# dscripka/openWakeWord

Measured on NVIDIA B200. Metric: 80ms audio-frames/sec (concurrent streams), higher is better.
Workload: dtype f16 operands / f32 accumulate (mel, BN, LayerNorm, sigmoid in f32; heads' first layer as fp16 hi/lo split = f32-grade)

## Files before the change

### openwakeword_b200/csrc/cnn_tc_inc.cu

```cuda
#include "oww_internal.h"
#include "tc_common.cuh"
#include "mel_device.cuh"
#include <cstring>

namespace {

constexpr int kIncEpiWarps = 16;
constexpr int kIncThreads = (kIncEpiWarps + 2) * 32;
constexpr int kIncAcc = 4;
constexpr int kIncMaxG = 7;
constexpr int kMelNF = 2;

__device__ __forceinline__ __half2 u32_as_half2(uint32_t v) {
    return __halves2half2(__ushort_as_half((unsigned short)(v & 0xFFFFu)), __ushort_as_half((unsigned short)(v >> 16)));
}
__device__ __forceinline__ bool elect_one() {
    uint32_t pred;
    asm volatile("{\n\t.reg .pred p;\n\telect.sync _|p, 0xffffffff;\n\tselp.u32 %0, 1, 0, p;\n\t}" : "=r"(pred));
    return pred != 0;
}
__device__ __forceinline__ void named_bar_sync(int id, int n) { asm volatile("bar.sync %0, %1;" ::"r"(id), "r"(n) : "memory"); }
__device__ __forceinline__ void tmem_ld8(uint32_t taddr, uint32_t* v) {
    asm volatile("tcgen05.ld.sync.aligned.32x32b.x8.b32 {%0,%1,%2,%3,%4,%5,%6,%7}, [%8];"
                 : "=r"(v[0]), "=r"(v[1]), "=r"(v[2]), "=r"(v[3]), "=r"(v[4]), "=r"(v[5]), "=r"(v[6]), "=r"(v[7])
// ... 184 lines not shown
                            for (int q = 0; q < nq; ++q) {
                                const uint32_t alo = (q < n_pair ? a_hi_pair : a_hi_self) | ((a_tap + (uint32_t)q * pitch2) & 0x3FFFu);
                                const uint32_t blo = b_lo0 | ((b_tap + (uint32_t)q * np2) & 0x3FFFu);
                                tc_mma_f16(d_tmem, dhi | alo, dhi | blo, idesc, accumulate);
                                accumulate = 1;
                            }
                        }
                        }
                        tc_commit(tfull(acc));
                    }
                    __syncwarp();
                    if (++acc == kIncAcc) { acc = 0; acc_par ^= 1; }
                }
                if (dbg) a.dbg_clock[41 + l] = clock64() - c0;
                have_prev = true; prev_i = i;
                __syncwarp();
            }
        }
    } else {
        const int et = threadIdx.x;
        const int quarter = warp & 3, part = warp >> 2;
        const int row = quarter * 32 + lane;
        int acc = 0; uint32_t acc_par = 0;
        uint32_t epar[2] = {0, 0};
        uint32_t epi_tails_par = 0;
        uint32_t hf_par = 0; int hchunk_e = 0;
        for (int grp = blockIdx.x; grp < P.n_groups; grp += gridDim.x) {
            const uint4* tin = a.tails_in + (int64_t)grp * P.tail_units;
            uint4* tout = a.tails_out + (int64_t)grp * P.tail_units;
            int* s_cnt = reinterpret_cast<int*>(smem + 512);
            int* s_live = s_cnt + 16;
            float* s_mel = reinterpret_cast<float*>(smem + P.scratch_off + 6144);
            if (a.dbg_clock && blockIdx.x == 0 && grp == 0 && et == 0) a.dbg_clock[101] = clock64();
            named_bar_sync(2, kIncEpiWarps * 32);
            if (et < G) {
                const int b = grp * G + et;
                s_live[et] = b < a.B;
            }
            named_bar_sync(2, kIncEpiWarps * 32);
            if (a.fused) {
                uint8_t* sc = smem + P.scratch_off;
                float2* s_tw = reinterpret_cast<float2*>(sc);
                float* s_win = reinterpret_cast<float*>(sc + 4096);
                uint8_t* s_work = smem + 2048 + warp * (kMelNF * kMelFrameScratch);
                float* s_floor = s_mel + G * 256;
                int seen_v = 1;
                for (int i = et; i < 512; i += kIncEpiWarps * 32) { s_tw[i] = a.mel_twiddle[i]; s_win[i] = a.mel_window[i]; }
                if (et < G) {
                    const int b = grp * G + et;
                    s_cnt[et] = s_live[et] ? a.mel_count_rw[b] : 0;
                    s_cnt[8 + et] = s_live[et] ? a.feat_count[b] : 0;
                    seen_v = s_live[et] ? a.seen[b] : 1;
                    s_live[8 + et] = s_live[et] && seen_v == 0;
                }
                named_bar_sync(2, kIncEpiWarps * 32);
                const int my_start = a.mel_start[lane], my_len = a.mel_len[lane];
                const float* my_w = a.mel_w + lane * OWW_MEL_MAXSUPPORT;
                for (int fi = warp * kMelNF; fi < G * 8; fi += kIncEpiWarps * kMelNF) {
                    const int16_t* tl[kMelNF]; const int16_t* bd[kMelNF]; int fr[kMelNF]; float db[kMelNF];
#pragma unroll
                    for (int i = 0; i < kMelNF; ++i) {
                        const int fj = fi + i < G * 8 ? fi + i : fi;
                        int b = grp * G + (fj >> 3);
                        if (b >= a.B) b = grp * G;
                        tl[i] = a.tail + (int64_t)b * OWW_TAIL; bd[i] = a.pcm + (int64_t)b * a.pcm_stride; fr[i] = fj & 7;
                    }
                    long long* st = (a.dbg_clock && blockIdx.x == 0 && grp == 0 && warp == 0 && fi == 0) ? a.dbg_clock + 92 : nullptr;
                    mel_frames_db<kMelNF>(tl, OWW_TAIL, bd, fr, s_work, s_tw, s_win, a.mel_kmax, my_start, my_len, my_w, lane, db, st);
#pragma unroll
                    for (int i = 0; i < kMelNF; ++i)
                        if (fi + i < G * 8) s_mel[(fi + i) * 32 + lane] = db[i];
                }
                named_bar_sync(2, kIncEpiWarps * 32);
                if (a.dbg_clock && blockIdx.x == 0 && grp == 0 && et == 0) a.dbg_clock[97] = clock64();
                constexpr int kTW = OWW_TAIL / 2;
                const bool al = ((size_t)a.pcm & 3) == 0 && (a.pcm_stride & 1) == 0;
                uint32_t tv[4]; int ti[4];
#pragma unroll
                for (int u = 0; u < 4; ++u) {
                    const int i = et + u * kIncEpiWarps * 32;
                    ti[u] = -1; tv[u] = 0;
                    if (i < G * kTW) {
                        const int g = i / kTW, k = i - g * kTW, b = grp * G + g;
                        if (s_live[g]) {
                            const int16_t* src = a.pcm + (int64_t)b * a.pcm_stride + (OWW_SAMPLES_PER_CHUNK - OWW_TAIL) + 2 * k;
                            tv[u] = al ? __ldg(reinterpret_cast<const uint32_t*>(src))
                                       : ((uint32_t)(unsigned short)__ldg(src) | ((uint32_t)(unsigned short)__ldg(src + 1) << 16));
                            ti[u] = b * kTW + k;
// ... 859 lines not shown
```

### openwakeword_b200/csrc/mel_device.cuh

```cuda
#pragma once
#include <cuda_runtime.h>
#include <cstdint>
#include "oww_internal.h"

namespace {

__device__ __forceinline__ float2 cmul(float2 a, float2 b) {
    return make_float2(__fmaf_rn(a.x, b.x, -__fmul_rn(a.y, b.y)), __fmaf_rn(a.x, b.y, __fmul_rn(a.y, b.x)));
}

template <bool kBodyGlobal = true>
__device__ __forceinline__ float mel_frame_db(const int16_t* tail, int prefix, const int16_t* body, int f, float2* a, float2* b,
                                              float* pw_buf, const float2* s_tw, const float* s_win, int kmax, int my_start,
                                              int my_len, const float* my_w, int lane) {
#pragma unroll
        for (int j = 0; j < 8; ++j) {
            const int n = lane + 32 * j;
            const int s0 = f * OWW_HOP + 2 * n;
            float x0, x1;
            if (s0 + 1 < prefix) { x0 = (float)tail[s0]; x1 = (float)tail[s0 + 1]; }
            else if (s0 >= prefix) {
                if (kBodyGlobal) { x0 = (float)__ldg(body + (s0 - prefix)); x1 = (float)__ldg(body + (s0 + 1 - prefix)); }
                else { x0 = (float)body[s0 - prefix]; x1 = (float)body[s0 + 1 - prefix]; }
            }
// ... 67 lines not shown
                                              uint8_t* bufs, const float2* s_tw, const float* s_win, int kmax, int my_start,
                                              int my_len, const float* my_w, int lane, float* db, long long* stamps = nullptr) {
    float2* a[NF]; float2* b[NF]; float* pw[NF];
    if (stamps && lane == 0) stamps[0] = clock64();
#pragma unroll
    for (int i = 0; i < NF; ++i) {
        a[i] = reinterpret_cast<float2*>(bufs + i * kMelFrameScratch);
        b[i] = a[i] + 256;
        pw[i] = reinterpret_cast<float*>(b[i] + 256);
    }
    bool al[NF];
#pragma unroll
    for (int i = 0; i < NF; ++i) al[i] = (((size_t)body[i] | (size_t)tail[i]) & 3) == 0 && (prefix & 1) == 0;
    uint32_t raw[8][NF];
#pragma unroll
    for (int j = 0; j < 8; ++j) {
        const int n = lane + 32 * j;
#pragma unroll
        for (int i = 0; i < NF; ++i) {
            const int s0 = f[i] * OWW_HOP + 2 * n;
            if (al[i]) {
                raw[j][i] = s0 + 1 < prefix ? *reinterpret_cast<const uint32_t*>(tail[i] + s0)
                                            : __ldg(reinterpret_cast<const uint32_t*>(body[i] + (s0 - prefix)));
            } else {
                unsigned short u0, u1;
                if (s0 + 1 < prefix) { u0 = (unsigned short)tail[i][s0]; u1 = (unsigned short)tail[i][s0 + 1]; }
                else if (s0 >= prefix) { u0 = (unsigned short)__ldg(body[i] + (s0 - prefix)); u1 = (unsigned short)__ldg(body[i] + (s0 + 1 - prefix)); }
                else { u0 = (unsigned short)tail[i][s0]; u1 = (unsigned short)__ldg(body[i]); }
                raw[j][i] = (uint32_t)u0 | ((uint32_t)u1 << 16);
            }
        }
    }
#pragma unroll
    for (int j = 0; j < 8; ++j) {
        const int n = lane + 32 * j;
        const float2 wn = *reinterpret_cast<const float2*>(s_win + 2 * n);
#pragma unroll
        for (int i = 0; i < NF; ++i) {
            const float x0 = (float)(short)(raw[j][i] & 0xFFFFu), x1 = (float)(short)(raw[j][i] >> 16);
            a[i][fswz(n)] = make_float2(__fmul_rn(x0, wn.x), __fmul_rn(x1, wn.y));
        }
    }
    __syncwarp();
    if (stamps && lane == 0) stamps[1] = clock64();
#pragma unroll
    for (int Ns = 1; Ns < 256; Ns *= 4) {
        const int tstep = 128 / Ns;
        float2 t1 = make_float2(1.f, 0.f), t2 = t1, t3 = t1;
        if (Ns > 1 && Ns <= 32) { const int k = lane & (Ns - 1); t1 = s_tw[k * tstep]; t2 = s_tw[2 * k * tstep]; t3 = s_tw[3 * k * tstep]; }
#pragma unroll
        for (int jj = 0; jj < 2; ++jj) {
            const int j = lane + 32 * jj;
            const int k = j & (Ns - 1);
            if (Ns > 32) { t1 = s_tw[k * tstep]; t2 = s_tw[2 * k * tstep]; t3 = s_tw[3 * k * tstep]; }
            const int dst = (j / Ns) * Ns * 4 + k;
            const int sj = fswz(j);
            const int d0 = fswz(dst), d1 = fswz(dst + Ns), d2 = fswz(dst + 2 * Ns), d3 = fswz(dst + 3 * Ns);
#pragma unroll
            for (int i = 0; i < NF; ++i) {
                const float2 v0 = a[i][sj];
                float2 v1 = a[i][sj + 64], v2 = a[i][sj + 128], v3 = a[i][sj + 192];
                if (Ns > 1) { v1 = cmul(v1, t1); v2 = cmul(v2, t2); v3 = cmul(v3, t3); }
                float2 a0 = make_float2(v0.x + v2.x, v0.y + v2.y);
                float2 a1 = make_float2(v0.x - v2.x, v0.y - v2.y);
                float2 a2 = make_float2(v1.x + v3.x, v1.y + v3.y);
                float2 d = make_float2(v1.x - v3.x, v1.y - v3.y);
                float2 a3 = make_float2(d.y, -d.x);
                b[i][d0] = make_float2(a0.x + a2.x, a0.y + a2.y);
                b[i][d1] = make_float2(a1.x + a3.x, a1.y + a3.y);
                b[i][d2] = make_float2(a0.x - a2.x, a0.y - a2.y);
                b[i][d3] = make_float2(a1.x - a3.x, a1.y - a3.y);
            }
        }
        __syncwarp();
#pragma unroll
        for (int i = 0; i < NF; ++i) { float2* t = a[i]; a[i] = b[i]; b[i] = t; }
    }
    if (stamps && lane == 0) stamps[2] = clock64();
    for (int k = lane; k < kmax; k += 32) {
#pragma unroll
        for (int i = 0; i < NF; ++i) {
            float p;
            if (k == 256) {
                const float x = a[i][fswz(0)].x - a[i][fswz(0)].y;
                p = __fmul_rn(x, x);
            } else {
                const float2 zk = a[i][fswz(k & 255)];
                const float2 zc = a[i][fswz((256 - k) & 255)];
                const float2 xe = make_float2(0.5f * (zk.x + zc.x), 0.5f * (zk.y - zc.y));
                const float2 dd = make_float2(zk.x - zc.x, zk.y + zc.y);
                const float2 xo = make_float2(0.5f * dd.y, -0.5f * dd.x);
                const float2 t2 = cmul(s_tw[k], xo);
                const float re = __fadd_rn(xe.x, t2.x), im = __fadd_rn(xe.y, t2.y);
                p = __fmaf_rn(re, re, __fmul_rn(im, im));
            }
// ... 26 lines not shown
```

### openwakeword_b200/csrc/api.cu

```cuda
#include "oww_internal.h"
#include <cstdarg>
#include <cstdlib>
#include <cstring>
#include <algorithm>

static thread_local std::string g_create_error;

int oww_fail(oww_ctx* ctx, int code, const char* fmt, ...) {
    char buf[512];
    va_list ap;
    va_start(ap, fmt);
    vsnprintf(buf, sizeof(buf), fmt, ap);
    va_end(ap);
    if (ctx) ctx->err = buf; else g_create_error = buf;
    return code;
}

namespace {

const int kLayerTable[OWW_N_CONV][6] = {
    {3, 3, 1, 24, 0, 0},
    {1, 3, 24, 24, 0, 0}, {3, 1, 24, 24, 2, 2},
    {1, 3, 24, 48, 0, 0}, {3, 1, 48, 48, 0, 0},
    {1, 3, 48, 48, 0, 0}, {3, 1, 48, 48, 1, 2},
// ... 139 lines not shown
        const int r = (int)((i / 24) % n_rows);
        const int64_t clip = i / ((int64_t)24 * n_rows);
        reinterpret_cast<float4*>(feats + clip * clip_stride + (int64_t)r * 96)[c4] =
            init ? __ldg(reinterpret_cast<const float4*>(init + (int64_t)r * 96) + c4) : make_float4(0.f, 0.f, 0.f, 0.f);
    }
}

int ensure_emb_tmp(oww_ctx* ctx, size_t floats) {
    if (ctx->emb_tmp_floats >= floats) return OWW_OK;
    cudaFree(ctx->d_emb_tmp); ctx->d_emb_tmp = nullptr; ctx->emb_tmp_floats = 0;
    OWW_CUDA(ctx, cudaMalloc(&ctx->d_emb_tmp, floats * sizeof(float)));
    ctx->emb_tmp_floats = floats;
    return OWW_OK;
}

int step_core(oww_ctx* ctx, const int16_t* d_pcm, int64_t pcm_stride, int n_chunks, float* d_scores, int out_stride,
              cudaStream_t s) {
    const int B = ctx->n_streams;
    if (B <= 0) return oww_fail(ctx, OWW_EINVAL, "oww_set_streams has not been called");
    if (n_chunks < 1 || n_chunks > ctx->cfg.max_chunks)
        return oww_fail(ctx, OWW_EINVAL, "n_chunks=%d outside [1,%d]", n_chunks, ctx->cfg.max_chunks);
    if (!ctx->mel_loaded || !ctx->emb_loaded) return oww_fail(ctx, OWW_EINVAL, "weights not loaded");
    int rc;
    const long slot = ctx->timing ? ctx->ev_steps % ctx->ev_slots : 0;
    cudaEvent_t* ev = ctx->timing ? &ctx->ev[4 * slot] : nullptr;
    const bool inc = ctx->cfg.cnn_mode == OWW_CNN_TC_INCREMENTAL;
    const FeatSrc fs0{ctx->d_feat_ring, (int64_t)ctx->feat_rows * 96, ctx->d_feat_count, ctx->feat_rows - 1, 0};

    if (inc && n_chunks == 1 && oww_fused_frontend_supported(ctx)) {
        const bool heads_inside = oww_fused_heads_supported(ctx);
        if (ev) OWW_CUDA(ctx, cudaEventRecord(ev[1], s));
        if ((rc = oww_fused_step(ctx, d_pcm, pcm_stride, d_scores, out_stride, heads_inside, s))) return rc;
        if (ctx->late_active) {
            if ((rc = oww_late_chain(ctx, ctx->d_emb_tmp, s))) return rc;
            if ((rc = oww_feat_append(ctx, ctx->d_emb_tmp, 1, s))) return rc;
        }
        if (ev) OWW_CUDA(ctx, cudaEventRecord(ev[2], s));
        if (heads_inside) oww_feat16_invalidate(ctx);
        else if ((rc = oww_feat16_advance(ctx, 1, s))) return rc;
        if (!heads_inside && (rc = oww_heads_all(ctx, fs0, B, d_scores, out_stride, 0, s))) return rc;
        if (ev) {
            if (heads_inside) ctx->ev_fused[slot] = 1;
            else { OWW_CUDA(ctx, cudaEventRecord(ev[3], s)); ctx->ev_fused[slot] = 2; }
            ctx->ev_steps++;
        }
        return OWW_OK;
    }

    if (ev) { OWW_CUDA(ctx, cudaEventRecord(ev[0], s)); ctx->ev_fused[slot] = 0; }
    MelLaunch m{d_pcm, pcm_stride, n_chunks * OWW_SAMPLES_PER_CHUNK, ctx->d_tail, ctx->d_seen, ctx->d_mel_ring,
                (int64_t)ctx->mel_rows * 32, ctx->mel_rows - 1, ctx->d_mel_count, B, 1, n_chunks};
    if ((rc = oww_mel_launch(ctx, m, s))) return rc;
    if (ev) OWW_CUDA(ctx, cudaEventRecord(ev[1], s));
    WindowSrc ws{ctx->d_mel_ring, (int64_t)ctx->mel_rows * 32, ctx->d_mel_count, ctx->mel_rows - 1, B, n_chunks};
    if (inc) {
        for (int i = 0; i < n_chunks; ++i)
            if ((rc = oww_cnn_inc_step(ctx, 8 * (n_chunks - 1 - i), ctx->d_emb_tmp + (size_t)i * B * 96, s))) return rc;
    } else {
        if ((rc = oww_cnn_window(ctx, ws, B * n_chunks, ctx->d_emb_tmp, s, false))) return rc;
    }
    if ((rc = oww_feat_append(ctx, ctx->d_emb_tmp, n_chunks, s))) return rc;
    if (ev) OWW_CUDA(ctx, cudaEventRecord(ev[2], s));
    if ((rc = oww_feat16_advance(ctx, n_chunks, s))) return rc;
    for (int i = n_chunks - 1; i >= 0; --i) {
        FeatSrc fs = fs0; fs.back = i;
        if ((rc = oww_heads_all(ctx, fs, B, d_scores, out_stride, i != n_chunks - 1, s))) return rc;
    }
    if (ev) { OWW_CUDA(ctx, cudaEventRecord(ev[3], s)); ctx->ev_steps++; }
// ... 648 lines not shown
```

### openwakeword_b200/csrc/cnn_tc.cu

```cuda
#include "oww_internal.h"
#include "tc_common.cuh"
#include <cmath>
#include <cstring>

namespace {

struct Tc0Args {
    WindowSrc src;
    int n_windows; int T_out;
    const float* w; const float* scale; const float* bias;
    __half* out; int64_t plane;
};

__global__ void __launch_bounds__(256) tc_conv0_kernel(Tc0Args a) {
    __shared__ float s_w[9 * 24];
    __shared__ float s_s[24], s_b[24];
    for (int i = threadIdx.x; i < 9 * 24; i += 256) s_w[i] = a.w[i];
    if (threadIdx.x < 24) { s_s[threadIdx.x] = a.scale[threadIdx.x]; s_b[threadIdx.x] = a.bias[threadIdx.x]; }
    __syncthreads();
    constexpr int Wp = 33;
    const int T = a.T_out;
    const int64_t total = (int64_t)a.n_windows * T * Wp;
    for (int64_t p = (int64_t)blockIdx.x * 256 + threadIdx.x; p < total; p += (int64_t)gridDim.x * 256) {
        const int f = (int)(p % Wp);
// ... 269 lines not shown
                    if (po == 0) o[(int64_t)g * a.out_plane - 1] = make_uint4(0, 0, 0, 0);
                    if (a.out_split) {
                        o[(int64_t)(a.cg_out + g) * a.out_plane] = *reinterpret_cast<uint4*>(l);
                        if (po == 0) o[(int64_t)(a.cg_out + g) * a.out_plane - 1] = make_uint4(0, 0, 0, 0);
                    }
#pragma unroll
                    for (int kk = 0; kk < 2; ++kk)
                        if (a.out_b[kk]) {
                            uint4* ob = reinterpret_cast<uint4*>(a.out_b[kk]) + kGuard + (int64_t)n * a.out_T * Wp +
                                        (int64_t)(t + a.out_b_toff[kk]) * Wp + f;
                            ob[(int64_t)g * a.out_plane] = *reinterpret_cast<uint4*>(h);
                            if (a.out_split) ob[(int64_t)(a.cg_out + g) * a.out_plane] = *reinterpret_cast<uint4*>(l);
                        }
                }
            }
        }
    }
    tc_fence_before();
    __syncthreads();
    if (warp == 1) {
        tc_fence_after();
        asm volatile("tcgen05.dealloc.cta_group::1.sync.aligned.b32 %0, %1;" ::"r"(tmem_base), "r"(256));
    }
}

struct TcBlkArgs {
    const __half* in; LateLay lay;
    const __half* w; const float* scale; const float* bias;
    int n, W, rows_new;
    int m_valid, tap;
    int pool_f;
    int cg_in, cg_out, apply_act, n_tiles;
    float* out_f32;
    __half* out[3]; int out_toff[3];
    LateLay out_lay;
    int64_t out_plane;
};

template <int CGP, int NP>
__global__ void __launch_bounds__(kTcThreads, 1) tc_conv_blk_kernel(TcBlkArgs a) {
    extern __shared__ __align__(128) uint8_t smem[];
    constexpr int W_TERM = 3 * CGP * NP * 16;
    constexpr int W_BYTES = 2 * W_TERM;
    uint8_t* w_smem = smem;
    const int units = a.lay.units;
    const int half_bytes = CGP * units * 16;
    uint8_t* a_smem = smem + W_BYTES;
    uint64_t* bars = reinterpret_cast<uint64_t*>(a_smem + 2 * half_bytes);
    uint32_t* tmem_slot = reinterpret_cast<uint32_t*>(bars + 4 + 2 * kAccStages + 1);
    float* s_sb = reinterpret_cast<float*>(tmem_slot + 4);
    for (int i = threadIdx.x; i < NP; i += kTcThreads) { s_sb[i] = a.scale[i]; s_sb[NP + i] = a.bias[i]; }

    const int warp = threadIdx.x >> 5, lane = threadIdx.x & 31;
    const uint32_t bar0 = smem_u32(bars);
    auto full_bar = [&](int h) { return bar0 + 8u * h; };
    auto empty_bar = [&](int h) { return bar0 + 8u * (2 + h); };
    auto tfull_bar = [&](int s) { return bar0 + 8u * (4 + s); };
    auto tempty_bar = [&](int s) { return bar0 + 8u * (4 + kAccStages + s); };
    const uint32_t wfull_bar = bar0 + 8u * (4 + 2 * kAccStages);

    if (threadIdx.x == 0) {
        for (int h = 0; h < 2; ++h) { mbar_init(full_bar(h), 1); mbar_init(empty_bar(h), 1); }
        for (int s = 0; s < kAccStages; ++s) { mbar_init(tfull_bar(s), 1); mbar_init(tempty_bar(s), 8); }
        mbar_init(wfull_bar, 1);
        asm volatile("fence.mbarrier_init.release.cluster;" ::: "memory");
    }
    if (a.cg_in < CGP)
        for (int h = 0; h < 2; ++h) {
            uint4* pz = reinterpret_cast<uint4*>(a_smem + h * half_bytes + a.cg_in * units * 16);
            for (int i = threadIdx.x; i < (CGP - a.cg_in) * units; i += kTcThreads) pz[i] = make_uint4(0, 0, 0, 0);
        }
    asm volatile("fence.proxy.async.shared::cta;" ::: "memory");
    if (warp == 1) {
        asm volatile("tcgen05.alloc.cta_group::1.sync.aligned.shared::cta.b32 [%0], %1;" ::"r"(smem_u32(tmem_slot)), "r"(256));
        asm volatile("tcgen05.relinquish_alloc_permit.cta_group::1.sync.aligned;");
    }
    tc_fence_before();
    __syncthreads();
    tc_fence_after();
    const uint32_t tmem_base = *tmem_slot;
    pdl_trigger();

    if (warp == 0) {
// ... 48 lines not shown
                    }
                    __syncwarp();
                }
                phase ^= 1;
                if (++acc == kAccStages) { acc = 0; acc_phase ^= 1; }
            }
        }
    } else {
        const int quarter = warp & 3, half = (warp - 2) >> 2;
        constexpr int NP8 = NP / 8, PH = NP8 / 2;
        const int pl0 = half * PH;
        const int row = quarter * 32 + lane;
        int t, sl, f;
        if (a.lay.kh3) { const int SW = a.lay.S * a.W; t = row / SW; sl = (row - t * SW) / a.W; f = row - t * SW - sl * a.W; }
        else { const int per = a.lay.T * a.lay.Wq; sl = row / per; t = (row - sl * per) / a.lay.Wq; f = row - sl * per - t * a.lay.Wq; }
        const bool row_ok = row < a.m_valid && f < a.W;
        pdl_wait();
        int acc = 0; uint32_t acc_phase = 0;
        for (int tile = blockIdx.x; tile < a.n_tiles; tile += gridDim.x) {
            mbar_wait(tfull_bar(acc), acc_phase);
            tc_fence_after();
            uint32_t v[PH * 8];
            const uint32_t taddr = tmem_base + ((uint32_t)(quarter * 32) << 16) + (uint32_t)acc * 128u + (uint32_t)pl0 * 8u;
#pragma unroll
            for (int k = 0; k < PH; ++k) tc_tmem_ld8(taddr + k * 8, v + k * 8);
            tmem_wait_ld();
            tc_fence_before();
            __syncwarp();
            if (lane == 0) mbar_arrive(tempty_bar(acc));
            if (++acc == kAccStages) { acc = 0; acc_phase ^= 1; }

            const int n = tile * a.lay.S + sl;
            const bool live = row_ok && n < a.n;
            if (a.out_f32) {
                if (!live || f != 0) continue;
                float* o = a.out_f32 + ((int64_t)n * a.rows_new + t) * 96;
#pragma unroll
                for (int k = 0; k < PH; ++k) {
                    const int c = (pl0 + k) * 8;
                    if (c >= 96) continue;
                    float4 r0, r1;
                    r0.x = fmaf(__uint_as_float(v[k * 8 + 0]), s_sb[c + 0], s_sb[NP + c + 0]);
                    r0.y = fmaf(__uint_as_float(v[k * 8 + 1]), s_sb[c + 1], s_sb[NP + c + 1]);
                    r0.z = fmaf(__uint_as_float(v[k * 8 + 2]), s_sb[c + 2], s_sb[NP + c + 2]);
                    r0.w = fmaf(__uint_as_float(v[k * 8 + 3]), s_sb[c + 3], s_sb[NP + c + 3]);
                    r1.x = fmaf(__uint_as_float(v[k * 8 + 4]), s_sb[c + 4], s_sb[NP + c + 4]);
                    r1.y = fmaf(__uint_as_float(v[k * 8 + 5]), s_sb[c + 5], s_sb[NP + c + 5]);
                    r1.z = fmaf(__uint_as_float(v[k * 8 + 6]), s_sb[c + 6], s_sb[NP + c + 6]);
                    r1.w = fmaf(__uint_as_float(v[k * 8 + 7]), s_sb[c + 7], s_sb[NP + c + 7]);
                    reinterpret_cast<float4*>(o + c)[0] = r0;
                    reinterpret_cast<float4*>(o + c)[1] = r1;
                }
                continue;
            }
            const bool pooled = a.pool_f == 2;
            const bool writer = live && (!pooled || (f & 1) == 0);
            const int fo = pooled ? f >> 1 : f;
            int64_t dst[3];
#pragma unroll
            for (int kk = 0; kk < 3; ++kk)
                dst[kk] = a.out_lay.S ? late_unit(a.out_lay, 0, live ? n : 0, t + a.out_toff[kk], fo)
                                      : kGuard + ((int64_t)(live ? n : 0) * a.rows_new + t) * (a.W + 1) + f;
            const int64_t pstride = a.out_lay.S ? (int64_t)a.out_lay.units : a.out_plane;
#pragma unroll
            for (int k = 0; k < PH; ++k) {
                const int g = pl0 + k;
                __half2 h[4], l[4];
#pragma unroll
                for (int u = 0; u < 4; ++u) {
                    const int c = g * 8 + u * 2;
                    float y0 = fmaf(__uint_as_float(v[k * 8 + u * 2]), s_sb[c], s_sb[NP + c]);
                    float y1 = fmaf(__uint_as_float(v[k * 8 + u * 2 + 1]), s_sb[c + 1], s_sb[NP + c + 1]);
                    if (a.apply_act) { y0 = act(y0); y1 = act(y1); }
                    if (pooled) {
                        y0 = fmaxf(y0, __shfl_xor_sync(0xffffffffu, y0, 1));
                        y1 = fmaxf(y1, __shfl_xor_sync(0xffffffffu, y1, 1));
                    }
                    const __half h0 = __float2half_rn(y0), h1 = __float2half_rn(y1);
                    h[u] = __halves2half2(h0, h1);
                    l[u] = __floats2half2_rn(y0 - __half2float(h0), y1 - __half2float(h1));
                }
                if (g >= a.cg_out || !writer) continue;
#pragma unroll
                for (int kk = 0; kk < 3; ++kk)
                    if (a.out[kk]) {
                        uint4* o = reinterpret_cast<uint4*>(a.out[kk]) + dst[kk];
                        o[(int64_t)g * pstride] = *reinterpret_cast<uint4*>(h);
                        o[(int64_t)(a.cg_out + g) * pstride] = *reinterpret_cast<uint4*>(l);
                    }
            }
        }
    }
    tc_fence_before();
    __syncthreads();
    if (warp == 1) {
        tc_fence_after();
        asm volatile("tcgen05.dealloc.cta_group::1.sync.aligned.b32 %0, %1;" ::"r"(tmem_base), "r"(256));
    }
}

struct PoolOut { __half* p[3]; int toff[3]; int out_T; LateLay lay = {0, 0, 0, 0, 0, 0}; };
__global__ void __launch_bounds__(256) tc_pool_kernel(const __half* in, int64_t in_plane, PoolOut po, int64_t out_plane,
                                                      int n, int t_in, int w_in, int cg, int pt, int pf, int split) {
    __half* const out = po.p[0];
    pdl_trigger();
    pdl_wait();
    const int t_out = t_in / pt, w_out = w_in / pf;
    const int wp_in = w_in + 1, wp_out = w_out + 1;
    const int64_t per_out = (int64_t)t_out * wp_out;
    const int64_t total = (int64_t)n * per_out * cg;
// ... 60 lines not shown
        const int f = (int)(r % w); r /= w;
        const int tt = (int)(r % t);
        const int64_t s = r / t;
        const int64_t p = s * (int64_t)t * wp + (int64_t)tt * wp + f;
        float v = __half2float(in[((int64_t)(ch >> 3) * plane + kGuard + p) * 8 + (ch & 7)]);
        if (split) v += __half2float(in[((int64_t)(c / 8 + (ch >> 3)) * plane + kGuard + p) * 8 + (ch & 7)]);
        out[i] = v;
    }
}

struct TcLayerGeom { int T, W, cg, cgp, np, T_out, rows, lo, tap_off[3]; };

inline int round8(int v) { return (v + 7) & ~7; }

template <int CGP, int NP, int TERMS>
int launch_tc(oww_ctx* ctx, const TcConvArgs& a, cudaStream_t s) {
    constexpr int split = TERMS == 3 ? 2 : 1, stages = TERMS == 3 ? 2 : 4;
    const size_t smem = (size_t)split * 3 * CGP * NP * 16 + (size_t)stages * split * CGP * a.rows * 16 +
                        8 * (2 * stages + 2 * kAccStages + 1) + 16 + 2 * NP * sizeof(float);
    if (smem > 227 * 1024) return oww_fail(ctx, OWW_EUNSUPPORTED, "tcgen05 conv tile does not fit shared memory (%zu bytes)", smem);
    const uint32_t bit = 1u << (((CGP / 2 + NP / 16) + (TERMS == 3 ? 16 : 0)) & 31);
    if (!(ctx->tc_attr_mask & bit)) {
        OWW_CUDA(ctx, cudaFuncSetAttribute(tc_conv_kernel<CGP, NP, TERMS>, cudaFuncAttributeMaxDynamicSharedMemorySize, 227 * 1024));
        ctx->tc_attr_mask |= bit;
    }
    int grid = ctx->sm_count < a.n_tiles ? ctx->sm_count : a.n_tiles;
    tc_conv_kernel<CGP, NP, TERMS><<<grid, kTcThreads, smem, s>>>(a);
    OWW_LAUNCH_CHECK(ctx);
    return OWW_OK;
}

template <int CGP, int NP>
int launch_tc_blk(oww_ctx* ctx, const TcBlkArgs& a, cudaStream_t s) {
    const size_t smem = (size_t)2 * 3 * CGP * NP * 16 + (size_t)2 * CGP * a.lay.units * 16 + 8 * (4 + 2 * kAccStages + 1) + 16 + 2 * NP * sizeof(float);
    if (smem > 227 * 1024) return oww_fail(ctx, OWW_EUNSUPPORTED, "blocked late conv tile does not fit shared memory (%zu bytes)", smem);
    const uint32_t bit = 1u << (CGP / 2);
    if (!(ctx->tc_blk_attr_mask & bit)) {
        OWW_CUDA(ctx, cudaFuncSetAttribute(tc_conv_blk_kernel<CGP, NP>, cudaFuncAttributeMaxDynamicSharedMemorySize, 227 * 1024));
        ctx->tc_blk_attr_mask |= bit;
    }
    const int grid = ctx->sm_count < a.n_tiles ? ctx->sm_count : a.n_tiles;
    cudaLaunchConfig_t cfg;
    std::memset(&cfg, 0, sizeof(cfg));
    cfg.gridDim = dim3(grid); cfg.blockDim = dim3(kTcThreads); cfg.dynamicSmemBytes = smem; cfg.stream = s;
    cudaLaunchAttribute at[1];
    at[0].id = cudaLaunchAttributeProgrammaticStreamSerialization;
    at[0].val.programmaticStreamSerializationAllowed = ctx->late_pdl ? 1 : 0;
    cfg.attrs = at; cfg.numAttrs = 1;
    OWW_CUDA(ctx, cudaLaunchKernelEx(&cfg, tc_conv_blk_kernel<CGP, NP>, a));
    OWW_LAUNCH_CHECK(ctx);
    return OWW_OK;
}

}

int oww_tc_pack_weights(oww_ctx* ctx, const float* h_blob) {
    size_t off = 0, total_h = 0, total_f = 0;
    for (int li = 1; li < OWW_N_CONV; ++li) {
        const ConvLayer& L = ctx->conv[li];
        const int cg = L.cin / 8, cgp = (cg + 1) & ~1, np = (L.cout + 15) & ~15;
        total_h += (size_t)3 * cgp * np * 8;
        total_f += 2 * (size_t)np;
    }
    std::vector<__half> hw(total_h), hw3(2 * total_h);
    std::vector<float> hf(total_f), hf3(total_f);
    size_t oh = 0, of = 0;
    for (int li = 0; li < OWW_N_CONV; ++li) {
// ... 216 lines not shown
            if (kh3) while (Y.S > 1 && X.T_buf * Y.S * W > 256) Y.S /= 2;
            const int tap = kh3 ? Y.S * W : 1;
            Y.units = round8(std::max((kh3 ? 0 : 1) + Y.T * Y.S * Y.Wq, 2 * tap + 128));
            Y.blk_stride = (int64_t)2 * X.cg * Y.units;
            buf_units = (size_t)((n + Y.S - 1) / Y.S) * Y.blk_stride;
            X.plane = 0;
        } else {
            X.plane = (int64_t)((kGuard + (int64_t)n * X.T_buf * (W + 1) + kGuardBack + 7) & ~7LL);
            buf_units = (size_t)2 * X.cg * X.plane;
        }
        X.tmpl_off = kh3 ? (int)tmpl_units : -1;
        if (kh3) tmpl_units += (size_t)2 * X.cg * 2 * (W + 1);
        for (int k = 0; k < X.n_buf; ++k) {
            OWW_CUDA(ctx, cudaMalloc(&X.buf[k], buf_units * 16));
            OWW_CUDA(ctx, cudaMemset(X.buf[k], 0, buf_units * 16));
        }
        if (C.pool_t) {
            const size_t u = (size_t)2 * (C.cout / 8) * ((kGuard + (size_t)n * rows * (W + 1) + kGuardBack + 7) & ~(size_t)7);
            if (u > tmp_units) tmp_units = u;
            rows /= C.pool_t; W /= C.pool_f;
        }
    }
    if (tmp_units) {
        OWW_CUDA(ctx, cudaMalloc(&ctx->d_late_tmp[0], tmp_units * 16));
        OWW_CUDA(ctx, cudaMemset(ctx->d_late_tmp[0], 0, tmp_units * 16));
    }
    OWW_CUDA(ctx, cudaMalloc(&ctx->d_late_template, std::max<size_t>(tmpl_units, 1) * 16));
    OWW_CUDA(ctx, cudaMemset(ctx->d_late_template, 0, std::max<size_t>(tmpl_units, 1) * 16));
    ctx->late_step = 0;
    ctx->late_active = true;
    return OWW_OK;
}

int oww_late_chain(oww_ctx* ctx, float* d_emb, cudaStream_t s) {
    const int L0 = ctx->split_from, n = ctx->n_streams;
    const long k = ctx->late_step;
    for (int l = L0; l < OWW_N_CONV; ++l) {
        const ConvLayer& C = ctx->conv[l];
        const oww_ctx::LateTensor& X = ctx->late_x[l];
        const bool last = l == OWW_N_CONV - 1;
        const int cg = C.cin / 8, cgp = (cg + 1) & ~1, np = (C.cout + 15) & ~15;
        const int W = X.W, Wp = W + 1, T = X.T_buf, T_out = X.rows_new;
        auto route = [&](const oww_ctx::LateTensor& Y, __half** p, int* toff, int& n_out) {
            n_out = 0;
            if (Y.n_buf == 1) { p[0] = reinterpret_cast<__half*>(Y.buf[0]); toff[0] = 0; n_out = 1; return; }
            const int r = Y.rows_new;
            for (int m = 0; m < Y.n_buf; ++m) {
                p[m] = reinterpret_cast<__half*>(Y.buf[(k + m) % Y.n_buf]);
                toff[m] = 2 - m * r;
            }
            n_out = Y.n_buf;
        };
        const int64_t tmp_plane = (int64_t)((kGuard + (int64_t)n * T_out * Wp + kGuardBack + 7) & ~7LL);
        int rc;
        bool pool_fused = false;
        if (X.lay.S) {
            TcBlkArgs b;
            std::memset(&b, 0, sizeof(b));
            b.in = reinterpret_cast<const __half*>(X.buf[X.n_buf == 1 ? 0 : (int)(k % X.n_buf)]);
            b.lay = X.lay;
            b.w = reinterpret_cast<const __half*>(ctx->d_tc_w3) + 2 * ctx->tc_w_off[l];
            b.scale = ctx->d_tc_sb3 + ctx->tc_sb_off[l]; b.bias = b.scale + np;
            b.n = n; b.W = W; b.rows_new = T_out;
            b.m_valid = T_out * X.lay.S * X.lay.Wq;
            b.tap = C.kh == 3 ? X.lay.S * W : 1;
            b.cg_in = cg; b.cg_out = C.cout / 8; b.apply_act = last ? 0 : 1;
            b.n_tiles = (n + X.lay.S - 1) / X.lay.S;
            const bool fuse_pool = !last && C.pool_t == 1 && C.pool_f == 2 && X.lay.kh3 && (W & 1) == 0 && ctx->late_x[l + 1].lay.S > 0;
            if (last) {
                b.out_f32 = d_emb;
            } else if (fuse_pool) {
                const oww_ctx::LateTensor& Y = ctx->late_x[l + 1];
                int n_out = 0;
                route(Y, b.out, b.out_toff, n_out);
                b.out_lay = Y.lay;
                b.pool_f = 2;
                pool_fused = true;
            } else if (C.pool_t) {
                b.out[0] = reinterpret_cast<__half*>(ctx->d_late_tmp[0]);
                b.out_plane = tmp_plane;
            } else {
                const oww_ctx::LateTensor& Y = ctx->late_x[l + 1];
                int n_out = 0;
                route(Y, b.out, b.out_toff, n_out);
                b.out_lay = Y.lay;
            }
            if (cgp == 12 && np == 96) rc = launch_tc_blk<12, 96>(ctx, b, s);
            else if (cgp == 10 && np == 96) rc = launch_tc_blk<10, 96>(ctx, b, s);
            else rc = oww_fail(ctx, OWW_EUNSUPPORTED, "no block-major late conv instance for cgp=%d np=%d", cgp, np);
            if (rc) return rc;
        } else {
        TcConvArgs a;
        std::memset(&a, 0, sizeof(a));
        a.in = reinterpret_cast<const __half*>(X.buf[X.n_buf == 1 ? 0 : (int)(k % X.n_buf)]);
        a.in_plane = X.plane;
        a.w = reinterpret_cast<const __half*>(ctx->d_tc_w3) + 2 * ctx->tc_w_off[l];
        a.scale = ctx->d_tc_sb3 + ctx->tc_sb_off[l]; a.bias = a.scale + np;
        a.n = n; a.T = T; a.W = W; a.T_out = T_out;
        if (C.kw == 3) { a.lo = 1; a.tap_off[0] = 0; a.tap_off[1] = 1; a.tap_off[2] = 2; a.rows = round8(128 + 2); }
        else { a.lo = 0; a.tap_off[0] = 0; a.tap_off[1] = Wp; a.tap_off[2] = 2 * Wp; a.rows = round8(128 + 2 * Wp); }
        a.cg_in = cg; a.cg_out = C.cout / 8; a.apply_act = last ? 0 : 1;
        a.p_in = (int64_t)n * T * Wp;
        a.n_tiles = (int)((a.p_in + 127) / 128);
// ... 55 lines not shown
```

### openwakeword_b200/csrc/oww_internal.h

```cpp
#pragma once
#include <cuda_runtime.h>
#include <cstdint>
#include <cstdio>
#include <string>
#include <utility>
#include <vector>
#include "owwb200.h"

#define OWW_N_CONV 20
#define OWW_FFT_N 512
#define OWW_N_BINS 257
#define OWW_HOP 160
#define OWW_TAIL 480
#define OWW_MEL_MAXSUPPORT 32

struct ConvLayer {
    int kh, kw, cin, cout, pool_t, pool_f;
    int t_in, f_in;
    int t_out, f_out;
    float* d_w;
    float* d_scale;
    float* d_bias;
};

// ... 209 lines not shown
            return oww_fail((ctx), OWW_ECUDA, "kernel launch failed: %s (%s:%d)",              \
                            cudaGetErrorString(e__), __FILE__, __LINE__);                      \
    } while (0)

struct MelLaunch {
    const int16_t* body; int64_t body_stride; int n_body;
    int16_t* tail;
    int* seen;
    float* out; int64_t out_stride; int out_rows_mask;
    int* out_count;
    int n_clips; int affine; int n_chunks;
    const int* ids = nullptr;
};
int oww_mel_launch(oww_ctx* ctx, const MelLaunch& p, cudaStream_t s);
int oww_mel_clips_launch(oww_ctx* ctx, const int16_t* d_pcm, int64_t clip_stride, int n_clips, int n_samples, int pad, int steps,
                         float* d_out, int64_t out_stride, cudaStream_t s);

struct WindowSrc {
    const float* base; int64_t stride;
    const int* count; int rows_mask;
    int n_streams; int n_chunks;
    const int* ids = nullptr;
};
int oww_cnn_clip_fp32(oww_ctx* ctx, const float* d_mel, int n, int T, float* d_emb, cudaStream_t s);
int oww_feat_append(oww_ctx* ctx, const float* d_emb, int n_chunks, cudaStream_t s, const int* d_ids = nullptr, int n_ids = 0);
int oww_cnn_window(oww_ctx* ctx, const WindowSrc& src, int n_windows, float* d_emb, cudaStream_t s, bool capture_tails = false);

int oww_tc_pack_weights(oww_ctx* ctx, const float* h_blob);
size_t oww_tc_act_units(const oww_ctx* ctx, int n_windows);
size_t oww_tc_act_units_T(const oww_ctx* ctx, int n, int T0);
int oww_cnn_tc_clip(oww_ctx* ctx, const float* d_mel, int n, int T, float* d_emb, cudaStream_t s);
int oww_cnn_tc_clip_rows(oww_ctx* ctx, const WindowSrc& src, int n, int T, float* d_emb, int out_rows, cudaStream_t s);
int oww_late_alloc(oww_ctx* ctx);
int oww_late_chain(oww_ctx* ctx, float* d_emb, cudaStream_t s);
int oww_late_capture(oww_ctx* ctx, int next_layer, const void* planes, int64_t plane_pitch, int T, int W, cudaStream_t s);
int oww_cnn_tc_pyramid(oww_ctx* ctx, const WindowSrc& src, int n, float* d_emb, int stop_layer, float* d_dbg, cudaStream_t s);
struct TailCapture { int win0, n_win, stream0; const int* ids = nullptr; bool late = false; };
int oww_cnn_tc_pyramid_cap(oww_ctx* ctx, const WindowSrc& src, int n, float* d_emb, const TailCapture* cap, cudaStream_t s);

int oww_inc_build_plan(oww_ctx* ctx, int G, int n_streams, int n_layers, IncPlan* out);
int oww_inc_n_layers(const oww_ctx* ctx);
int oww_inc_setup(oww_ctx* ctx, const float* h_blob);
int oww_inc_alloc_streams(oww_ctx* ctx);
int oww_cnn_inc_step(oww_ctx* ctx, int back, float* d_emb, cudaStream_t s);
bool oww_fused_frontend_supported(const oww_ctx* ctx);
bool oww_fused_heads_supported(const oww_ctx* ctx);
int oww_fused_step(oww_ctx* ctx, const int16_t* d_pcm, int64_t pcm_stride, float* d_scores, int out_stride, bool with_heads,
                   cudaStream_t s);
int oww_heads_sync_devs(oww_ctx* ctx);
int oww_inc_capture(oww_ctx* ctx, int layer, const void* planes, int64_t plane_pitch, int T, int W, int win0, int n_win,
                    int stream0, const int* d_ids, cudaStream_t s);
int oww_cnn_fp32_pyramid(oww_ctx* ctx, const WindowSrc& src, int n, float* d_emb, int stop_layer, float* d_dbg, cudaStream_t s);

struct FeatSrc {
    const float* base; int64_t stride;
    const int* count; int rows_mask;
    int back;
    int steps = 0, row0 = 0;
};
int oww_heads_launch(oww_ctx* ctx, int head_id, const FeatSrc& src, int n, float* d_out, int out_stride,
                     int out_col0, int combine_max, cudaStream_t s, uint32_t head_mask = 0xFFFFFFFFu);

int oww_heads_tc_pack(oww_ctx* ctx, Head& h, const float* w1);
bool oww_heads_tc_supported(const oww_ctx* ctx, int head_id);
int oww_heads_tc_launch(oww_ctx* ctx, int head_id, const FeatSrc& src, int n, float* d_out, int out_stride,
                        int out_col0, int combine_max, cudaStream_t s, uint32_t head_mask = 0xFFFFFFFFu);
void oww_heads_grp_free(oww_ctx* ctx);
// ... 9 lines not shown
```

Baseline: 10.52 million.

## Fuse windowing into first radix-4 FFT stage and merge mel setup barriers

The windowing pass now directly computes the first (twiddle-free) radix-4 butterfly from register-held samples and writes to the ping-pong buffer. This removes one full shared-memory write/read round trip and a warp sync per frame. Separately, the per-group setup loads twiddles, window values and per-stream counters into registers before a barrier, then publishes them in one pass, which drops one named barrier per group. Register pressure rises slightly, and the new setup relies on exactly 512 epilogue threads.

Measured after the change: 10.69 million, median of 6. 1.02x the previous value.

```diff
diff --git a/openwakeword_b200/csrc/cnn_tc_inc.cu b/openwakeword_b200/csrc/cnn_tc_inc.cu
--- a/openwakeword_b200/csrc/cnn_tc_inc.cu
+++ b/openwakeword_b200/csrc/cnn_tc_inc.cu
@@ -240,28 +240,32 @@
             int* s_live = s_cnt + 16;
             float* s_mel = reinterpret_cast<float*>(smem + P.scratch_off + 6144);
             if (a.dbg_clock && blockIdx.x == 0 && grp == 0 && et == 0) a.dbg_clock[101] = clock64();
-            named_bar_sync(2, kIncEpiWarps * 32);
-            if (et < G) {
-                const int b = grp * G + et;
-                s_live[et] = b < a.B;
+            static_assert(kIncEpiWarps * 32 == 512, "one twiddle and one window value per epilogue thread");
+            const bool live = et < G && grp * G + et < a.B;
+            int cnt_mel = 0, cnt_feat = 0, seen_v = 1;
+            float2 tw_v = make_float2(0.f, 0.f); float win_v = 0.f;
+            if (a.fused) {
+                tw_v = a.mel_twiddle[et]; win_v = a.mel_window[et];
+                if (live) {
+                    const int b = grp * G + et;
+                    cnt_mel = a.mel_count_rw[b]; cnt_feat = a.feat_count[b]; seen_v = a.seen[b];
+                }
             }
             named_bar_sync(2, kIncEpiWarps * 32);
+            uint8_t* sc = smem + P.scratch_off;
+            float2* s_tw = reinterpret_cast<float2*>(sc);
+            float* s_win = reinterpret_cast<float*>(sc + 4096);
+            if (et < G) {
+                s_live[et] = live;
+                s_cnt[et] = cnt_mel;
+                s_cnt[8 + et] = cnt_feat;
+                s_live[8 + et] = live && seen_v == 0;
+            }
+            if (a.fused) { s_tw[et] = tw_v; s_win[et] = win_v; }
+            named_bar_sync(2, kIncEpiWarps * 32);
             if (a.fused) {
-                uint8_t* sc = smem + P.scratch_off;
-                float2* s_tw = reinterpret_cast<float2*>(sc);
-                float* s_win = reinterpret_cast<float*>(sc + 4096);
                 uint8_t* s_work = smem + 2048 + warp * (kMelNF * kMelFrameScratch);
                 float* s_floor = s_mel + G * 256;
-                int seen_v = 1;
-                for (int i = et; i < 512; i += kIncEpiWarps * 32) { s_tw[i] = a.mel_twiddle[i]; s_win[i] = a.mel_window[i]; }
-                if (et < G) {
-                    const int b = grp * G + et;
-                    s_cnt[et] = s_live[et] ? a.mel_count_rw[b] : 0;
-                    s_cnt[8 + et] = s_live[et] ? a.feat_count[b] : 0;
-                    seen_v = s_live[et] ? a.seen[b] : 1;
-                    s_live[8 + et] = s_live[et] && seen_v == 0;
-                }
-                named_bar_sync(2, kIncEpiWarps * 32);
                 const int my_start = a.mel_start[lane], my_len = a.mel_len[lane];
                 const float* my_w = a.mel_w + lane * OWW_MEL_MAXSUPPORT;
                 for (int fi = warp * kMelNF; fi < G * 8; fi += kIncEpiWarps * kMelNF) {
diff --git a/openwakeword_b200/csrc/mel_device.cuh b/openwakeword_b200/csrc/mel_device.cuh
--- a/openwakeword_b200/csrc/mel_device.cuh
+++ b/openwakeword_b200/csrc/mel_device.cuh
@@ -123,22 +123,41 @@
         }
     }
 #pragma unroll
-    for (int j = 0; j < 8; ++j) {
-        const int n = lane + 32 * j;
-        const float2 wn = *reinterpret_cast<const float2*>(s_win + 2 * n);
+    for (int jj = 0; jj < 2; ++jj) {
+        const int j = lane + 32 * jj;
+        float2 wn[4];
+#pragma unroll
+        for (int m = 0; m < 4; ++m) wn[m] = *reinterpret_cast<const float2*>(s_win + 2 * (j + 64 * m));
+        const int d0 = fswz(4 * j), d1 = fswz(4 * j + 1), d2 = fswz(4 * j + 2), d3 = fswz(4 * j + 3);
 #pragma unroll
         for (int i = 0; i < NF; ++i) {
-            const float x0 = (float)(short)(raw[j][i] & 0xFFFFu), x1 = (float)(short)(raw[j][i] >> 16);
-            a[i][fswz(n)] = make_float2(__fmul_rn(x0, wn.x), __fmul_rn(x1, wn.y));
+            float2 v[4];
+#pragma unroll
+            for (int m = 0; m < 4; ++m) {
+                const uint32_t r = raw[jj + 2 * m][i];
+                const float x0 = (float)(short)(r & 0xFFFFu), x1 = (float)(short)(r >> 16);
+                v[m] = make_float2(__fmul_rn(x0, wn[m].x), __fmul_rn(x1, wn[m].y));
+            }
+            const float2 a0 = make_float2(v[0].x + v[2].x, v[0].y + v[2].y);
+            const float2 a1 = make_float2(v[0].x - v[2].x, v[0].y - v[2].y);
+            const float2 a2 = make_float2(v[1].x + v[3].x, v[1].y + v[3].y);
+            const float2 d = make_float2(v[1].x - v[3].x, v[1].y - v[3].y);
+            const float2 a3 = make_float2(d.y, -d.x);
+            b[i][d0] = make_float2(a0.x + a2.x, a0.y + a2.y);
+            b[i][d1] = make_float2(a1.x + a3.x, a1.y + a3.y);
+            b[i][d2] = make_float2(a0.x - a2.x, a0.y - a2.y);
+            b[i][d3] = make_float2(a1.x - a3.x, a1.y - a3.y);
         }
     }
     __syncwarp();
+#pragma unroll
+    for (int i = 0; i < NF; ++i) { float2* t = a[i]; a[i] = b[i]; b[i] = t; }
     if (stamps && lane == 0) stamps[1] = clock64();
 #pragma unroll
-    for (int Ns = 1; Ns < 256; Ns *= 4) {
+    for (int Ns = 4; Ns < 256; Ns *= 4) {
         const int tstep = 128 / Ns;
-        float2 t1 = make_float2(1.f, 0.f), t2 = t1, t3 = t1;
-        if (Ns > 1 && Ns <= 32) { const int k = lane & (Ns - 1); t1 = s_tw[k * tstep]; t2 = s_tw[2 * k * tstep]; t3 = s_tw[3 * k * tstep]; }
+        float2 t1, t2, t3;
+        if (Ns <= 32) { const int k = lane & (Ns - 1); t1 = s_tw[k * tstep]; t2 = s_tw[2 * k * tstep]; t3 = s_tw[3 * k * tstep]; }
 #pragma unroll
         for (int jj = 0; jj < 2; ++jj) {
             const int j = lane + 32 * jj;
@@ -151,7 +170,7 @@
             for (int i = 0; i < NF; ++i) {
                 const float2 v0 = a[i][sj];
                 float2 v1 = a[i][sj + 64], v2 = a[i][sj + 128], v3 = a[i][sj + 192];
-                if (Ns > 1) { v1 = cmul(v1, t1); v2 = cmul(v2, t2); v3 = cmul(v3, t3); }
+                v1 = cmul(v1, t1); v2 = cmul(v2, t2); v3 = cmul(v3, t3);
                 float2 a0 = make_float2(v0.x + v2.x, v0.y + v2.y);
                 float2 a1 = make_float2(v0.x - v2.x, v0.y - v2.y);
                 float2 a2 = make_float2(v1.x + v3.x, v1.y + v3.y);
```

## Fuse 2x2 pooling and feature-ring append into blocked late conv epilogue

Applied to the files above, without the earlier changes.

The final late conv layer now writes its fp32 embedding directly into the per-stream feature ring and bumps the ring count in the epilogue, so the separate feat_append launch is skipped. A 2x2 max-pool case (pool_t=2, pool_f=2, W=2, T_out=2) is also fused into the epilogue, using a shared-memory exchange between warp quarters plus named barriers. The epilogue first computes scale, bias, activation and pooling into a register array, and extra shared memory is reserved for the exchange. This removes kernel launches and an intermediate pass, at the cost of added barriers, more registers and more shared memory.

New measurement: 10.46 million before, 10.56 million after (median of 6 runs). No clear change (+1.0%).

```diff
diff --git a/openwakeword_b200/csrc/api.cu b/openwakeword_b200/csrc/api.cu
--- a/openwakeword_b200/csrc/api.cu
+++ b/openwakeword_b200/csrc/api.cu
@@ -195,8 +195,9 @@
         if (ev) OWW_CUDA(ctx, cudaEventRecord(ev[1], s));
         if ((rc = oww_fused_step(ctx, d_pcm, pcm_stride, d_scores, out_stride, heads_inside, s))) return rc;
         if (ctx->late_active) {
-            if ((rc = oww_late_chain(ctx, ctx->d_emb_tmp, s))) return rc;
-            if ((rc = oww_feat_append(ctx, ctx->d_emb_tmp, 1, s))) return rc;
+            bool appended = false;
+            if ((rc = oww_late_chain(ctx, ctx->d_emb_tmp, s, true, &appended))) return rc;
+            if (!appended && (rc = oww_feat_append(ctx, ctx->d_emb_tmp, 1, s))) return rc;
         }
         if (ev) OWW_CUDA(ctx, cudaEventRecord(ev[2], s));
         if (heads_inside) oww_feat16_invalidate(ctx);
diff --git a/openwakeword_b200/csrc/cnn_tc.cu b/openwakeword_b200/csrc/cnn_tc.cu
--- a/openwakeword_b200/csrc/cnn_tc.cu
+++ b/openwakeword_b200/csrc/cnn_tc.cu
@@ -325,6 +325,7 @@
     int pool_f;
     int cg_in, cg_out, apply_act, n_tiles;
     float* out_f32;
+    float* ring; int64_t ring_stride; int ring_mask; int* count;
     __half* out[3]; int out_toff[3];
     LateLay out_lay;
     int64_t out_plane;
@@ -342,6 +343,7 @@
     uint64_t* bars = reinterpret_cast<uint64_t*>(a_smem + 2 * half_bytes);
     uint32_t* tmem_slot = reinterpret_cast<uint32_t*>(bars + 4 + 2 * kAccStages + 1);
     float* s_sb = reinterpret_cast<float*>(tmem_slot + 4);
+    float* xch = s_sb + 2 * NP;
     for (int i = threadIdx.x; i < NP; i += kTcThreads) { s_sb[i] = a.scale[i]; s_sb[NP + i] = a.bias[i]; }
 
     const int warp = threadIdx.x >> 5, lane = threadIdx.x & 31;
@@ -456,34 +458,62 @@
 
             const int n = tile * a.lay.S + sl;
             const bool live = row_ok && n < a.n;
-            if (a.out_f32) {
-                if (!live || f != 0) continue;
-                float* o = a.out_f32 + ((int64_t)n * a.rows_new + t) * 96;
-#pragma unroll
-                for (int k = 0; k < PH; ++k) {
-                    const int c = (pl0 + k) * 8;
-                    if (c >= 96) continue;
-                    float4 r0, r1;
-                    r0.x = fmaf(__uint_as_float(v[k * 8 + 0]), s_sb[c + 0], s_sb[NP + c + 0]);
-                    r0.y = fmaf(__uint_as_float(v[k * 8 + 1]), s_sb[c + 1], s_sb[NP + c + 1]);
-                    r0.z = fmaf(__uint_as_float(v[k * 8 + 2]), s_sb[c + 2], s_sb[NP + c + 2]);
-                    r0.w = fmaf(__uint_as_float(v[k * 8 + 3]), s_sb[c + 3], s_sb[NP + c + 3]);
-                    r1.x = fmaf(__uint_as_float(v[k * 8 + 4]), s_sb[c + 4], s_sb[NP + c + 4]);
-                    r1.y = fmaf(__uint_as_float(v[k * 8 + 5]), s_sb[c + 5], s_sb[NP + c + 5]);
-                    r1.z = fmaf(__uint_as_float(v[k * 8 + 6]), s_sb[c + 6], s_sb[NP + c + 6]);
-                    r1.w = fmaf(__uint_as_float(v[k * 8 + 7]), s_sb[c + 7], s_sb[NP + c + 7]);
-                    reinterpret_cast<float4*>(o + c)[0] = r0;
-                    reinterpret_cast<float4*>(o + c)[1] = r1;
+            if (a.out_f32 || a.ring) {
+                if (live && f == 0) {
+                    float* o = a.ring ? a.ring + (int64_t)n * a.ring_stride + (int64_t)((a.count[n] + t) & a.ring_mask) * 96
+                                      : a.out_f32 + ((int64_t)n * a.rows_new + t) * 96;
+#pragma unroll
+                    for (int k = 0; k < PH; ++k) {
+                        const int c = (pl0 + k) * 8;
+                        if (c >= 96) continue;
+                        float4 r0, r1;
+                        r0.x = fmaf(__uint_as_float(v[k * 8 + 0]), s_sb[c + 0], s_sb[NP + c + 0]);
+                        r0.y = fmaf(__uint_as_float(v[k * 8 + 1]), s_sb[c + 1], s_sb[NP + c + 1]);
+                        r0.z = fmaf(__uint_as_float(v[k * 8 + 2]), s_sb[c + 2], s_sb[NP + c + 2]);
+                        r0.w = fmaf(__uint_as_float(v[k * 8 + 3]), s_sb[c + 3], s_sb[NP + c + 3]);
+                        r1.x = fmaf(__uint_as_float(v[k * 8 + 4]), s_sb[c + 4], s_sb[NP + c + 4]);
+                        r1.y = fmaf(__uint_as_float(v[k * 8 + 5]), s_sb[c + 5], s_sb[NP + c + 5]);
+                        r1.z = fmaf(__uint_as_float(v[k * 8 + 6]), s_sb[c + 6], s_sb[NP + c + 6]);
+                        r1.w = fmaf(__uint_as_float(v[k * 8 + 7]), s_sb[c + 7], s_sb[NP + c + 7]);
+                        reinterpret_cast<float4*>(o + c)[0] = r0;
+                        reinterpret_cast<float4*>(o + c)[1] = r1;
+                    }
+                }
+                if (a.ring) {
+                    asm volatile("bar.sync 1, 256;" ::: "memory");
+                    if (live && f == 0 && t == 0 && half == 0) a.count[n] = oww_wrap_count(a.count[n] + a.rows_new);
                 }
                 continue;
             }
-            const bool pooled = a.pool_f == 2;
-            const bool writer = live && (!pooled || (f & 1) == 0);
-            const int fo = pooled ? f >> 1 : f;
+            const bool pooled = a.pool_f != 0;
+            float y[PH * 8];
+#pragma unroll
+            for (int e = 0; e < PH * 8; ++e) {
+                const int c = pl0 * 8 + e;
+                y[e] = fmaf(__uint_as_float(v[e]), s_sb[c], s_sb[NP + c]);
+                if (a.apply_act) y[e] = act(y[e]);
+                if (pooled) y[e] = fmaxf(y[e], __shfl_xor_sync(0xffffffffu, y[e], 1));
+            }
+            if (a.pool_f == 4) {
+                if (quarter >= 2 && (lane & 1) == 0) {
+                    float* x = xch + ((quarter - 2) * 16 + (lane >> 1)) * NP + pl0 * 8;
+#pragma unroll
+                    for (int e = 0; e < PH * 8; ++e) x[e] = y[e];
+                }
+                asm volatile("bar.sync 1, 256;" ::: "memory");
+                if (quarter < 2 && (lane & 1) == 0) {
+                    const float* x = xch + (quarter * 16 + (lane >> 1)) * NP + pl0 * 8;
+#pragma unroll
+                    for (int e = 0; e < PH * 8; ++e) y[e] = fmaxf(y[e], x[e]);
+                }
+                asm volatile("bar.sync 2, 256;" ::: "memory");
+            }
+            const bool writer = live && (!pooled || (f & 1) == 0) && (a.pool_f != 4 || t == 0);
+            const int fo = pooled ? f >> 1 : f, to = a.pool_f == 4 ? t >> 1 : t;
             int64_t dst[3];
 #pragma unroll
             for (int kk = 0; kk < 3; ++kk)
-                dst[kk] = a.out_lay.S ? late_unit(a.out_lay, 0, live ? n : 0, t + a.out_toff[kk], fo)
+                dst[kk] = a.out_lay.S ? late_unit(a.out_lay, 0, live ? n : 0, to + a.out_toff[kk], fo)
                                       : kGuard + ((int64_t)(live ? n : 0) * a.rows_new + t) * (a.W + 1) + f;
             const int64_t pstride = a.out_lay.S ? (int64_t)a.out_lay.units : a.out_plane;
 #pragma unroll
@@ -492,14 +522,7 @@
                 __half2 h[4], l[4];
 #pragma unroll
                 for (int u = 0; u < 4; ++u) {
-                    const int c = g * 8 + u * 2;
-                    float y0 = fmaf(__uint_as_float(v[k * 8 + u * 2]), s_sb[c], s_sb[NP + c]);
-                    float y1 = fmaf(__uint_as_float(v[k * 8 + u * 2 + 1]), s_sb[c + 1], s_sb[NP + c + 1]);
-                    if (a.apply_act) { y0 = act(y0); y1 = act(y1); }
-                    if (pooled) {
-                        y0 = fmaxf(y0, __shfl_xor_sync(0xffffffffu, y0, 1));
-                        y1 = fmaxf(y1, __shfl_xor_sync(0xffffffffu, y1, 1));
-                    }
+                    const float y0 = y[k * 8 + u * 2], y1 = y[k * 8 + u * 2 + 1];
                     const __half h0 = __float2half_rn(y0), h1 = __float2half_rn(y1);
                     h[u] = __halves2half2(h0, h1);
                     l[u] = __floats2half2_rn(y0 - __half2float(h0), y1 - __half2float(h1));
@@ -626,7 +649,8 @@
 
 template <int CGP, int NP>
 int launch_tc_blk(oww_ctx* ctx, const TcBlkArgs& a, cudaStream_t s) {
-    const size_t smem = (size_t)2 * 3 * CGP * NP * 16 + (size_t)2 * CGP * a.lay.units * 16 + 8 * (4 + 2 * kAccStages + 1) + 16 + 2 * NP * sizeof(float);
+    const size_t smem = (size_t)2 * 3 * CGP * NP * 16 + (size_t)2 * CGP * a.lay.units * 16 + 8 * (4 + 2 * kAccStages + 1) + 16 + 2 * NP * sizeof(float) +
+                        (size_t)32 * NP * sizeof(float);
     if (smem > 227 * 1024) return oww_fail(ctx, OWW_EUNSUPPORTED, "blocked late conv tile does not fit shared memory (%zu bytes)", smem);
     const uint32_t bit = 1u << (CGP / 2);
     if (!(ctx->tc_blk_attr_mask & bit)) {
@@ -909,9 +933,10 @@
     return OWW_OK;
 }
 
-int oww_late_chain(oww_ctx* ctx, float* d_emb, cudaStream_t s) {
+int oww_late_chain(oww_ctx* ctx, float* d_emb, cudaStream_t s, bool ring_append, bool* appended) {
     const int L0 = ctx->split_from, n = ctx->n_streams;
     const long k = ctx->late_step;
+    if (appended) *appended = false;
     for (int l = L0; l < OWW_N_CONV; ++l) {
         const ConvLayer& C = ctx->conv[l];
         const oww_ctx::LateTensor& X = ctx->late_x[l];
@@ -943,9 +968,24 @@
             b.tap = C.kh == 3 ? X.lay.S * W : 1;
             b.cg_in = cg; b.cg_out = C.cout / 8; b.apply_act = last ? 0 : 1;
             b.n_tiles = (n + X.lay.S - 1) / X.lay.S;
-            const bool fuse_pool = !last && C.pool_t == 1 && C.pool_f == 2 && X.lay.kh3 && (W & 1) == 0 && ctx->late_x[l + 1].lay.S > 0;
+            const bool next_blk = !last && ctx->late_x[l + 1].lay.S > 0;
+            const bool fuse_pool = next_blk && C.pool_t == 1 && C.pool_f == 2 && X.lay.kh3 && (W & 1) == 0;
+            const bool fuse_pool22 = next_blk && C.pool_t == 2 && C.pool_f == 2 && X.lay.kh3 && W == 2 && T_out == 2 && X.lay.S * W == 64;
             if (last) {
-                b.out_f32 = d_emb;
+                if (ring_append) {
+                    b.ring = ctx->d_feat_ring; b.ring_stride = (int64_t)ctx->feat_rows * 96; b.ring_mask = ctx->feat_rows - 1;
+                    b.count = ctx->d_feat_count;
+                    if (appended) *appended = true;
+                } else {
+                    b.out_f32 = d_emb;
+                }
+            } else if (fuse_pool22) {
+                const oww_ctx::LateTensor& Y = ctx->late_x[l + 1];
+                int n_out = 0;
+                route(Y, b.out, b.out_toff, n_out);
+                b.out_lay = Y.lay;
+                b.pool_f = 4;
+                pool_fused = true;
             } else if (fuse_pool) {
                 const oww_ctx::LateTensor& Y = ctx->late_x[l + 1];
                 int n_out = 0;
diff --git a/openwakeword_b200/csrc/oww_internal.h b/openwakeword_b200/csrc/oww_internal.h
--- a/openwakeword_b200/csrc/oww_internal.h
+++ b/openwakeword_b200/csrc/oww_internal.h
@@ -265,7 +265,7 @@
 int oww_cnn_tc_clip(oww_ctx* ctx, const float* d_mel, int n, int T, float* d_emb, cudaStream_t s);
 int oww_cnn_tc_clip_rows(oww_ctx* ctx, const WindowSrc& src, int n, int T, float* d_emb, int out_rows, cudaStream_t s);
 int oww_late_alloc(oww_ctx* ctx);
-int oww_late_chain(oww_ctx* ctx, float* d_emb, cudaStream_t s);
+int oww_late_chain(oww_ctx* ctx, float* d_emb, cudaStream_t s, bool ring_append = false, bool* appended = nullptr);
 int oww_late_capture(oww_ctx* ctx, int next_layer, const void* planes, int64_t plane_pitch, int T, int W, cudaStream_t s);
 int oww_cnn_tc_pyramid(oww_ctx* ctx, const WindowSrc& src, int n, float* d_emb, int stop_layer, float* d_dbg, cudaStream_t s);
 struct TailCapture { int win0, n_win, stream0; const int* ids = nullptr; bool late = false; };
```
